# bqqbarbhg/rtk

Measured on AMD Instinct MI355X. Metric: Mrays/sec (primary, closest-hit) on 1M-tri scene, higher is better.
Workload: dtype f32; 1 GPU; config2: 1M-tri soup (seed 1, spread 0.02), 4096x4096 coherent pinhole primary rays; bvh=gpu-lbvh, bvh_nodes=462584, launch=persistent, ray_order=as given, parallelism=ray-batch shards x1, BVH replicated

## Files before the change

include/rtk_amd.h:

```cpp
#ifndef RTK_AMD_H
#define RTK_AMD_H

#include "rtk.h"

#ifdef __cplusplus
extern "C" {
#endif

enum {
	RTK_AMD_OK = 0,
	RTK_AMD_ERR_NO_DEVICE = -1,
	RTK_AMD_ERR_BAD_ARG = -2,
	RTK_AMD_ERR_OOM = -3,
	RTK_AMD_ERR_HIP = -4,
	RTK_AMD_ERR_BAD_SCENE = -5,
	RTK_AMD_ERR_UNSUPPORTED = -6,
};

const char *rtk_amd_last_error(void);
int rtk_amd_device_count(void);
int rtk_amd_set_device(int device);

typedef struct rtk_dev_scene rtk_dev_scene;

// ... 122 lines not shown
int rtk_dev_trace_status(const rtk_dev_scene *ds, void *stream);

int rtk_dev_detect_image(const rtk_dev_scene *ds, const rtk_ray *d_rays, size_t n, uint32_t *width, uint32_t *height, void *stream);

int rtk_dev_trace_rays_counted(const rtk_dev_scene *ds, const rtk_ray *d_rays, size_t n,
	rtk_hit_record *d_hits, const rtk_trace_opts *opts, rtk_trace_counters *out);

int rtk_dev_trace_rays_any_counted(const rtk_dev_scene *ds, const rtk_ray *d_rays, size_t n,
	uint8_t *d_occluded, const rtk_trace_opts *opts, rtk_trace_counters *out);

typedef struct rtk_packet_counters {
	uint64_t tiles;
	uint64_t pairs;
	uint64_t node_steps;
	uint64_t triangles_fetched;
	uint64_t triangle_group_tests;
	uint64_t tiles_handed_back;
	uint64_t handed_back_node_steps;
	uint64_t handed_back_triangle_steps;
} rtk_packet_counters;
int rtk_dev_trace_rays_packet_counted(const rtk_dev_scene *ds, const rtk_ray *d_rays, size_t n,
	rtk_hit_record *d_hits, const rtk_trace_opts *opts, rtk_packet_counters *out);

typedef struct rtk_mgpu rtk_mgpu;
void rtk_amd_shard_range(size_t n, int rank, int num_shards, size_t *first, size_t *count);
rtk_mgpu *rtk_mgpu_create(const int *devices, int num_devices);
void rtk_mgpu_destroy(rtk_mgpu *m);
int rtk_mgpu_num_devices(const rtk_mgpu *m);
const rtk_dev_scene *rtk_mgpu_scene(const rtk_mgpu *m, int index);
int rtk_mgpu_build(rtk_mgpu *m, const rtk_scene_desc *desc);
int rtk_mgpu_upload(rtk_mgpu *m, const rtk_scene *scene);
int rtk_mgpu_refit(rtk_mgpu *m, const rtk_scene_desc *desc);
int rtk_mgpu_refit_meshes(rtk_mgpu *m, const rtk_scene_desc *desc, const uint32_t *mesh_ids, size_t num_ids);
int rtk_mgpu_trace_rays(rtk_mgpu *m, const rtk_ray *rays, size_t n, rtk_hit_record *records, const rtk_trace_opts *opts);
int rtk_mgpu_trace_rays_device(rtk_mgpu *m, const rtk_ray *const *d_rays, const size_t *counts, rtk_hit_record *const *d_records,
	rtk_hit_record *d_gathered, int root_index, const rtk_trace_opts *opts);
int rtk_mgpu_trace_rays_device_striped(rtk_mgpu *m, const rtk_ray *const *d_rays, const size_t *counts, rtk_hit_record *const *d_records,
	rtk_hit_record *const *d_striped, const rtk_trace_opts *opts);
void rtk_mgpu_striped_segment(const size_t *counts, int num_shards, int shard, int stripe, size_t *first, size_t *count);

size_t rtk_trace_rays(const rtk_scene *scene, const rtk_ray *rays, size_t n, rtk_hit *hits, uint8_t *hit_mask);
size_t rtk_trace_rays_filter(const rtk_scene *scene, const rtk_ray *rays, size_t n, rtk_hit *hits, uint8_t *hit_mask,
	rtk_filter_fn *filter, void *filter_user);
void rtk_amd_forget_scene(const rtk_scene *scene);

#ifdef __cplusplus
// ... 4 lines not shown
```

rtk_amd/api.py:

```python
import ctypes as C
import os

import numpy as np

from .types import (HIT_DTYPE, HIT_RECORD_DTYPE, RAY_DTYPE, MeshSet, SceneDesc, SceneHeader)

HERE = os.path.dirname(os.path.abspath(__file__))
LIB_PATH = os.environ.get("RTK_AMD_LIB") or os.path.join(HERE, "librtk_amd.so")

RTK_TRACE_STATIC = 1
RTK_TRACE_NO_PACKET = 2
RTK_TRACE_SORT_RAYS = 4
RTK_TRACE_EXACT_NODES = 8
RTK_TRACE_NO_ASM = 16


class RtkError(RuntimeError):
    pass


class SceneInfo(C.Structure):
    _fields_ = [("num_triangles", C.c_uint64), ("num_meshes", C.c_uint64), ("num_nodes", C.c_uint64),
                ("node_bytes", C.c_uint64), ("triangle_bytes", C.c_uint64), ("total_device_bytes", C.c_uint64),
                ("max_depth", C.c_uint32), ("stack_entries", C.c_uint32), ("build_ms", C.c_double)]
# ... 49 lines not shown
    _fields_ = [("tiles", C.c_uint64), ("pairs", C.c_uint64), ("node_steps", C.c_uint64), ("triangles_fetched", C.c_uint64),
                ("triangle_group_tests", C.c_uint64), ("tiles_handed_back", C.c_uint64),
                ("handed_back_node_steps", C.c_uint64), ("handed_back_triangle_steps", C.c_uint64)]

    def as_dict(self):
        return {k: int(getattr(self, k)) for k, _ in self._fields_}


RTK_H_SYMBOLS = ["rtk_start_build", "rtk_run_task", "rtk_get_build_size", "rtk_finish_build_to",
                 "rtk_finish_build", "rtk_build_scene", "rtk_free_scene", "rtk_trace_ray", "rtk_trace_ray_filter"]
RTK_AMD_H_SYMBOLS = ["rtk_amd_last_error", "rtk_amd_device_count", "rtk_amd_set_device",
                     "rtk_dev_scene_upload", "rtk_dev_scene_build", "rtk_dev_scene_free", "rtk_dev_scene_get_info",
                     "rtk_dev_scene_mesh_base", "rtk_dev_scene_primitive_order", "rtk_dev_scene_export_size", "rtk_dev_scene_export",
                     "rtk_dev_trace_rays", "rtk_dev_trace_rays_any", "rtk_dev_expand_hits",
                     "rtk_dev_trace_rays_counted", "rtk_dev_trace_rays_any_counted", "rtk_dev_trace_rays_packet_counted", "rtk_dev_detect_image", "rtk_trace_rays", "rtk_amd_forget_scene",
                     "rtk_dev_scene_validate", "rtk_amd_release_workspace", "rtk_dev_scene_upload_buffer",
                     "rtk_dev_trace_rays_filtered", "rtk_dev_trace_rays_any_filtered", "rtk_dev_trace_status",
                     "rtk_trace_rays_filter", "rtk_amd_shard_range", "rtk_mgpu_create", "rtk_mgpu_destroy", "rtk_mgpu_num_devices",
                     "rtk_mgpu_scene", "rtk_mgpu_build", "rtk_mgpu_upload", "rtk_mgpu_trace_rays", "rtk_mgpu_trace_rays_device",
                     "rtk_amd_set_builder", "rtk_amd_get_builder", "rtk_amd_set_per_ray",
                     "rtk_mgpu_trace_rays_device_striped", "rtk_mgpu_striped_segment",
                     "rtk_dev_scene_refit", "rtk_dev_scene_last_refit_ms", "rtk_mgpu_refit",
                     "rtk_dev_scene_refit_meshes", "rtk_dev_scene_last_refit_nodes", "rtk_mgpu_refit_meshes",
                     "rtk_dev_scene_quality"]

_lib = None


def lib():
    global _lib
    if _lib is not None:
        return _lib
    if not os.path.exists(LIB_PATH):
        raise RtkError("%s not found: build it with `make -C rtk_amd/csrc` (or __graft_entry__.build()); "
                       "there is no CPU fallback" % LIB_PATH)
    import torch
    L = C.CDLL(LIB_PATH)
    L.rtk_amd_last_error.restype = C.c_char_p
    L.rtk_amd_device_count.restype = C.c_int
    L.rtk_amd_set_device.argtypes = [C.c_int]
    L.rtk_dev_scene_upload.restype = C.c_void_p
    L.rtk_dev_scene_upload.argtypes = [C.c_void_p]
    L.rtk_dev_scene_build.restype = C.c_void_p
    L.rtk_dev_scene_build.argtypes = [C.POINTER(SceneDesc)]
    L.rtk_dev_scene_free.argtypes = [C.c_void_p]
    L.rtk_dev_scene_get_info.argtypes = [C.c_void_p, C.POINTER(SceneInfo)]
    L.rtk_dev_scene_mesh_base.argtypes = [C.c_void_p, C.c_void_p, C.c_size_t]
    L.rtk_dev_scene_primitive_order.restype = C.c_longlong
    L.rtk_dev_scene_primitive_order.argtypes = [C.c_void_p, C.c_void_p, C.c_size_t]
    L.rtk_dev_scene_export_size.restype = C.c_size_t
    L.rtk_dev_scene_export_size.argtypes = [C.c_void_p]
    L.rtk_dev_scene_export.restype = C.c_void_p
    L.rtk_dev_scene_export.argtypes = [C.c_void_p, C.c_void_p, C.c_size_t]
    L.rtk_dev_trace_rays.argtypes = [C.c_void_p, C.c_void_p, C.c_size_t, C.c_void_p, C.POINTER(TraceOpts), C.c_void_p]
    L.rtk_dev_trace_rays_any.argtypes = [C.c_void_p, C.c_void_p, C.c_size_t, C.c_void_p, C.POINTER(TraceOpts), C.c_void_p]
    L.rtk_dev_expand_hits.argtypes = [C.c_void_p, C.c_void_p, C.c_size_t, C.c_void_p, C.c_void_p, C.c_void_p]
    L.rtk_dev_trace_rays_packet_counted.argtypes = [C.c_void_p, C.c_void_p, C.c_size_t, C.c_void_p, C.POINTER(TraceOpts), C.POINTER(PacketCounters)]
    L.rtk_dev_trace_rays_counted.argtypes = [C.c_void_p, C.c_void_p, C.c_size_t, C.c_void_p, C.POINTER(TraceOpts),
                                             C.POINTER(TraceCounters)]
    L.rtk_dev_trace_rays_any_counted.argtypes = [C.c_void_p, C.c_void_p, C.c_size_t, C.c_void_p, C.POINTER(TraceOpts),
                                                 C.POINTER(TraceCounters)]
    L.rtk_trace_rays.restype = C.c_size_t
    L.rtk_trace_rays.argtypes = [C.c_void_p, C.c_void_p, C.c_size_t, C.c_void_p, C.c_void_p]
    L.rtk_amd_forget_scene.argtypes = [C.c_void_p]
    L.rtk_dev_scene_validate.argtypes = [C.c_void_p, C.POINTER(SceneCheck)]
    L.rtk_dev_scene_upload_buffer.restype = C.c_void_p
    L.rtk_dev_scene_upload_buffer.argtypes = [C.c_void_p, C.c_size_t]
    L.rtk_dev_trace_rays_filtered.argtypes = [C.c_void_p, C.c_void_p, C.c_size_t, C.c_void_p, C.POINTER(DevFilter),
                                              C.POINTER(TraceOpts), C.c_void_p]
    L.rtk_dev_trace_rays_any_filtered.argtypes = [C.c_void_p, C.c_void_p, C.c_size_t, C.c_void_p, C.POINTER(DevFilter),
                                                  C.POINTER(TraceOpts), C.c_void_p]
    L.rtk_dev_trace_status.argtypes = [C.c_void_p, C.c_void_p]
    L.rtk_trace_rays_filter.restype = C.c_size_t
    L.rtk_trace_rays_filter.argtypes = [C.c_void_p, C.c_void_p, C.c_size_t, C.c_void_p, C.c_void_p, C.c_void_p, C.c_void_p]
    L.rtk_amd_shard_range.restype = None
    L.rtk_amd_shard_range.argtypes = [C.c_size_t, C.c_int, C.c_int, C.POINTER(C.c_size_t), C.POINTER(C.c_size_t)]
    L.rtk_mgpu_create.restype = C.c_void_p
    L.rtk_mgpu_create.argtypes = [C.POINTER(C.c_int), C.c_int]
    L.rtk_mgpu_destroy.restype = None
    L.rtk_mgpu_destroy.argtypes = [C.c_void_p]
# ... 309 lines not shown
        torch = _torch()
        if hasattr(rays, "data_ptr"):
            d_rays, n = rays, rays.numel() * rays.element_size() // 32
        else:
            rays = np.ascontiguousarray(rays)
            n = rays.shape[0]
            d_rays = to_device(rays)
        d_rec = torch.empty(n * 16, dtype=torch.uint8, device="cuda")
        ctr = TraceCounters()
        torch.cuda.synchronize()
        _check(lib().rtk_dev_trace_rays_counted(self.handle, C.c_void_p(d_rays.data_ptr()), n, C.c_void_p(d_rec.data_ptr()),
                                                C.byref(opts) if opts is not None else None, C.byref(ctr)),
               "rtk_dev_trace_rays_counted")
        return d_rec.cpu().numpy().view(HIT_RECORD_DTYPE), ctr.as_dict()


    def detect_image(self, rays):
        rays = np.ascontiguousarray(rays)
        d_rays = to_device(rays)
        w, h = C.c_uint32(0), C.c_uint32(0)
        _check(lib().rtk_dev_detect_image(self.handle, C.c_void_p(d_rays.data_ptr()), C.c_size_t(rays.shape[0]), C.byref(w), C.byref(h), _stream_ptr()), "rtk_dev_detect_image")
        return int(w.value), int(h.value)

    def trace_packet_counted(self, rays, opts):
        torch = _torch()
        if hasattr(rays, "data_ptr"):
            d_rays, n = rays, rays.numel() * rays.element_size() // 32
        else:
            rays = np.ascontiguousarray(rays)
            n = rays.shape[0]
            d_rays = to_device(rays)
        d_rec = torch.empty(n * 16, dtype=torch.uint8, device="cuda")
        ctr = PacketCounters()
        torch.cuda.synchronize()
        _check(lib().rtk_dev_trace_rays_packet_counted(self.handle, C.c_void_p(d_rays.data_ptr()), n, C.c_void_p(d_rec.data_ptr()),
                                                       C.byref(opts) if opts is not None else None, C.byref(ctr)),
               "rtk_dev_trace_rays_packet_counted")
        return d_rec.cpu().numpy().view(HIT_RECORD_DTYPE), ctr.as_dict()



def build_scene(meshes):
    _torch()
    ms = meshes if isinstance(meshes, MeshSet) else MeshSet(meshes)
    p = lib().rtk_build_scene(C.byref(ms.desc))
    if not p:
# ... 51 lines not shown
```

rtk_amd/csrc/rtk_capi.hip:

```cpp
#include "rtk_dev.h"
#include "rtk_trace_plan.h"

#include <algorithm>
#include "rtk_layout_check.h"

#include <stdarg.h>
#include <stdio.h>
#include <stdlib.h>
#include <string.h>

#include <chrono>
#include <atomic>
#include <mutex>
#include <unordered_map>


static thread_local char g_error[512] = "";

void rtk_set_error(const char *fmt, ...)
{
	va_list ap;
	va_start(ap, fmt);
	vsnprintf(g_error, sizeof(g_error), fmt, ap);
	va_end(ap);
// ... 105 lines not shown
{
	if (!out) { rtk_set_error("rtk_dev_trace_rays_counted: NULL counters"); return RTK_AMD_ERR_BAD_ARG; }
	return rtk_launch_trace(ds, d_rays, n, d_hits, nullptr, opts, nullptr, false, out);
}

extern "C" int rtk_dev_trace_rays_any_counted(const rtk_dev_scene *ds, const rtk_ray *d_rays, size_t n,
	uint8_t *d_occluded, const rtk_trace_opts *opts, rtk_trace_counters *out)
{
	if (!out) { rtk_set_error("rtk_dev_trace_rays_any_counted: NULL counters"); return RTK_AMD_ERR_BAD_ARG; }
	return rtk_launch_trace(ds, d_rays, n, nullptr, d_occluded, opts, nullptr, true, out);
}

extern "C" int rtk_dev_trace_rays_packet_counted(const rtk_dev_scene *ds, const rtk_ray *d_rays, size_t n,
	rtk_hit_record *d_hits, const rtk_trace_opts *opts, rtk_packet_counters *out)
{
	if (!out) { rtk_set_error("rtk_dev_trace_rays_packet_counted: NULL counters"); return RTK_AMD_ERR_BAD_ARG; }
	return rtk_launch_trace(ds, d_rays, n, d_hits, nullptr, opts, nullptr, false, nullptr, nullptr, nullptr, nullptr, 0, out);
}

extern "C" int rtk_dev_detect_image(const rtk_dev_scene *ds, const rtk_ray *d_rays, size_t n, uint32_t *width, uint32_t *height, void *stream)
{
	if (!ds || !width || !height || (!d_rays && n)) { rtk_set_error("rtk_dev_detect_image: NULL argument"); return RTK_AMD_ERR_BAD_ARG; }
	return rtk_detect_image(ds, d_rays, n, (hipStream_t)stream, width, height);
}

extern "C" int rtk_dev_trace_status(const rtk_dev_scene *ds, void *stream)
{
	return rtk_trace_status(ds, (hipStream_t)stream);
}

extern "C" int rtk_dev_expand_hits(const rtk_dev_scene *ds, const rtk_hit_record *d_records, size_t n,
	rtk_hit *d_hits, uint8_t *d_mask, void *stream)
{
	return rtk_launch_expand(ds, d_records, n, d_hits, d_mask, (hipStream_t)stream);
}


namespace {

const size_t STRIPE = 4096;

uint64_t hash_words(const void *data, size_t n, uint64_t h)
{
	const unsigned char *p = static_cast<const unsigned char *>(data);
	size_t i = 0;
	for (; i + 8 <= n; i += 8) { uint64_t w; memcpy(&w, p + i, 8); h = (h ^ w) * 0x9e3779b97f4a7c15ull; h ^= h >> 29; }
// ... 555 lines not shown
```

rtk_amd/csrc/rtk_dev.h:

```cpp
#pragma once

#include <hip/hip_runtime.h>
#include <stdint.h>
#include <mutex>
#include <vector>

#include "rtk.h"
#include "rtk_amd.h"

#define RTK_MAX_DEVICES 64
#define RTK_REF_NONE 0xffffffffu
#define RTK_REF_LEAF 0x80000000u
#define RTK_TRI_LAST 1u
#define RTK_QUEUES 8
#define RTK_QUEUE_WORD(q) (16 + 16 * (q))
#define RTK_COUNTER_WORDS (16 + 16 * RTK_QUEUES)
#define RTK_ERROR_WORD RTK_COUNTER_WORDS

struct DevNode {
	float bx[2][4];
	float by[2][4];
	float bz[2][4];
	uint32_t child[4];
	uint32_t order[4];
// ... 155 lines not shown
	WorkspaceLoan() = default;
	WorkspaceLoan(const WorkspaceLoan &) = delete;
	WorkspaceLoan &operator=(const WorkspaceLoan &) = delete;
	~WorkspaceLoan() { release(); }
	bool take(int device, size_t bytes);
	void release();
};
bool rtk_is_device_ptr(const void *p);
static inline size_t rtk_padded(size_t bytes) { return ((bytes ? bytes : 1) + 255u) & ~(size_t)255u; }
void rtk_export_forget(const rtk_dev_scene *ds);
void rtk_sah_costs(float *cost_node, float *cost_tri);

size_t rtk_sort_scratch_words(uint32_t n);
bool rtk_sort_pairs_async(unsigned long long *keys_a, unsigned long long *keys_b, uint32_t *vals_a, uint32_t *vals_b,
	uint32_t n, uint32_t key_bits, uint32_t *scratch, hipStream_t stream);
bool rtk_sort_words_async(unsigned long long *keys_a, unsigned long long *keys_b, uint32_t n, uint32_t first_bit, uint32_t last_bit,
	uint32_t *scratch, hipStream_t stream);

int rtk_launch_trace(const rtk_dev_scene *ds, const rtk_ray *d_rays, size_t n, rtk_hit_record *d_hits,
	uint8_t *d_occluded, const rtk_trace_opts *opts, hipStream_t stream, bool any_hit, rtk_trace_counters *counted,
	const rtk_dev_filter *filter = nullptr, rtk_hit_record *d_cand = nullptr, uint32_t *d_cand_count = nullptr, uint32_t cand_k = 0,
	rtk_packet_counters *pk_counted = nullptr);
int rtk_detect_image(const rtk_dev_scene *ds, const rtk_ray *d_rays, size_t n, hipStream_t stream, uint32_t *w_out, uint32_t *h_out);
int rtk_trace_status(const rtk_dev_scene *ds, hipStream_t stream);
void rtk_scratch_free(LaunchScratch *s);
void rtk_scene_drop_stream(rtk_dev_scene *ds, hipStream_t stream);
int rtk_launch_trace_one(const rtk_dev_scene *ds, const rtk_ray *d_ray, rtk_hit *d_hit, uint8_t *d_mask, hipStream_t stream,
	unsigned long long *h_status, uint32_t ticket);
int rtk_launch_expand(const rtk_dev_scene *ds, const rtk_hit_record *d_records, size_t n, rtk_hit *d_hits,
	uint8_t *d_mask, hipStream_t stream, unsigned long long *h_status = nullptr, uint32_t ticket = 0);
```

rtk_amd/csrc/rtk_trace.hip:

```cpp
#include "rtk_dev.h"

#include <algorithm>
#include "rtk_trace_shared.h"

#include <math.h>
#include <stdio.h>
#include <stdlib.h>

#include <mutex>

#include "rtk_trace_lane.h"

#define RTK_PUSH(e_)                                                                                        \
	do {                                                                                                    \
		if (sp < LDS_STACK) { stk[sp][lane] = (e_); sp++; }                                                 \
		else if (sp - LDS_STACK < p.spill_cap) {                                                            \
			p.spill[(size_t)(sp - LDS_STACK) * p.spill_stride + glane] = (e_); sp++; if (COUNT) c_spills++; \
		} else p.counter[RTK_ERROR_WORD] = 1ull;                                                            \
	} while (0)

#define RTK_REF_RETRY 0xfffffffeu
#define RTK_POP()                                                                                           \
	do {                                                                                                    \
		if (sp == 0u) top = RTK_REF_NONE;                                                                   \
// ... 802 lines not shown
#include "rtk_lane_hot_image.h"

const TraceKnobs &rtk_trace_knobs()
{
	static const TraceKnobs knobs = [] {
		const auto env = [](const char *name, int value) { const char *v = getenv(name); return v ? atoi(v) : value; };
		TraceKnobs k;
		k.detect_image = env("RTK_AMD_DETECT_IMAGE", k.detect_image);
		k.tile_blocks = env("RTK_AMD_TILE_BLOCKS", k.tile_blocks);
		k.any_packets = env("RTK_AMD_ANY_PACKETS", k.any_packets);
		k.qnodes = env("RTK_AMD_QNODES", k.qnodes);
		k.packet_asm = env("RTK_AMD_PACKET_ASM", k.packet_asm);
		const int wanted = env("RTK_AMD_PACKET_BEAM", (int)k.packet_beam);
		k.packet_beam = wanted < 0 ? PacketKernel::Cpp : wanted > (int)PacketKernel::Beam2 ? PacketKernel::Beam2 : (PacketKernel)wanted;
		k.log_path = getenv("RTK_AMD_LOG_PATH") != nullptr;
		k.lane_asm = env("RTK_AMD_LANE_ASM", k.lane_asm);
		k.lane_lds = (size_t)env("RTK_AMD_LANE_LDS", (int)k.lane_lds);
		k.sort_cell_bits = (uint32_t)env("RTK_AMD_SORT_CELL_BITS", (int)k.sort_cell_bits);
		k.sort_octant = (uint32_t)env("RTK_AMD_SORT_OCTANT", (int)k.sort_octant);
		k.sort_key = env("RTK_AMD_SORT_KEY", k.sort_key);
		k.packet_entries = env("RTK_AMD_PACKET_ENTRIES", k.packet_entries);
		k.entry_target = (unsigned)env("RTK_AMD_ENTRY_TARGET", (int)k.entry_target);
		k.entry_levels = (unsigned)env("RTK_AMD_ENTRY_LEVELS", (int)k.entry_levels);
		k.hot_blocks_per_cu = env("RTK_AMD_HOT_BLOCKS_PER_CU", k.hot_blocks_per_cu);
		k.lane_stats = env("RTK_AMD_LANE_STATS", k.lane_stats);
		k.lane_blocks = env("RTK_AMD_LANE_BLOCKS", k.lane_blocks);
		return k;
	}();
	return knobs;
}

AsmModule &rtk_lane_module()
{
	static const AsmKernel table[2] = { { "rtk_lane_hot_closest", rtk_trace_knobs().lane_blocks }, { "rtk_lane_hot_any", 0 } };
	static AsmModule m(rtk_lane_hot_image, table, 2, "rtk_dev_trace: the assembly per-lane kernels are not loaded");
	return m;
}

const AsmModule::Loaded *AsmModule::on(int device)
{
	if (device < 0 || device >= RTK_MAX_DEVICES) return nullptr;
	std::lock_guard<std::mutex> lock(mutex);
	Loaded &h = slot[device];
	if (!h.tried) {
		int cur = -1;
		if (hipGetDevice(&cur) != hipSuccess || cur != device) return nullptr;
// ... 271 lines not shown
	const int occ = blocks_per_cu_of(ds->device, variant_of(rq, o, look_w, look_h, facts, kernels, knobs));
	const TracePlan plan = plan_trace(rq, o, look_w, look_h, facts, kernels, knobs, occ);
	if (plan.error != RTK_AMD_OK) { rtk_set_error("%s", plan.message); return plan.error; }
	if (knobs.log_path) fprintf(stderr, "rtk_dev_trace: n %zu image %u x %u packet %d hot %d beam %d opts %p flags %x\n", n, plan.image_w, plan.image_h, (int)plan.packet, (int)plan.hot, (int)plan.kernel, (const void *)opts, o.flags);
	p.dynamic = plan.dynamic;
	p.refill_min = plan.refill_min;
	p.node_exit = plan.node_exit;
	p.image_w = plan.image_w;
	p.image_h = plan.image_h;
	p.tile_blocks = plan.tile_blocks;

	std::lock_guard<std::mutex> lock(ds->scratch_mutex);
	LaunchScratch *sc = scratch_for(ds, stream);
	if (!sc) return RTK_AMD_ERR_OOM;
	int rc = grow_scratch(sc, plan, n, stream);
	if (rc != RTK_AMD_OK) return rc;
	p.spill = sc->d_spill;
	p.spill_stride = (uint32_t)(plan.spill_cap ? sc->spill_lanes : 0);
	p.spill_cap = (uint32_t)plan.spill_cap;
	p.counter = sc->d_counter;
	if (plan.sort_rays && (rc = enqueue_sort(ds, sc, d_rays, n, knobs, stream, &p.perm)) != RTK_AMD_OK) return rc;
	if ((plan.dynamic || plan.packet || counted) && !plan.entries) RTK_HIP_CHECK(hipMemsetAsync(sc->d_counter, 0, RTK_COUNTER_WORDS * sizeof(unsigned long long), stream), RTK_AMD_ERR_HIP);
	if (plan.entries) {
		rtk_packet_entries_launch(p, (PkBlockEntries *)sc->d_entries, ds->bound_abs > 1.0f ? ds->bound_abs : 1.0f, knobs.entry_target, knobs.entry_levels, stream);
		p.entries = (const PkBlockEntries *)sc->d_entries;
	}
	if (plan.hot) rc = enqueue_packet_hot(ds, sc, p, plan, any_hit, pk_counted != nullptr, stream);
	else if (plan.packet) rtk_packet_launch(p, (unsigned)plan.grid, stream, counted != nullptr);
	else if (plan.lane_hot) rc = enqueue_lane_hot(ds, sc, p, plan, any_hit, o.refill_given, knobs, stream);
	else hipLaunchKernelGGL(trace_variant(plan.variant), dim3((unsigned)plan.grid), dim3(BLOCK_THREADS), 0, stream, p);
	if (rc != RTK_AMD_OK) return rc;
	RTK_HIP_CHECK(hipGetLastError(), RTK_AMD_ERR_HIP);
	if (pk_counted && (rc = read_packet_counters(sc, n, stream, pk_counted)) != RTK_AMD_OK) return rc;
	if (counted) return read_counters(sc, stream, counted);
	return RTK_AMD_OK;
}

int rtk_trace_status(const rtk_dev_scene *ds_c, hipStream_t stream)
{
	rtk_dev_scene *ds = const_cast<rtk_dev_scene *>(ds_c);
	if (!ds) { rtk_set_error("rtk_dev_trace_status: NULL scene"); return RTK_AMD_ERR_BAD_ARG; }
	unsigned long long *word = nullptr;
	{
		std::lock_guard<std::mutex> lock(ds->scratch_mutex);
		for (LaunchScratch *s : ds->scratch) if (s->stream == stream) { word = s->d_counter + RTK_ERROR_WORD; break; }
	}
	if (!word) {
		RTK_HIP_CHECK(hipStreamSynchronize(stream), RTK_AMD_ERR_HIP);
		return RTK_AMD_OK;
	}
	unsigned long long e = 0;
	RTK_HIP_CHECK(hipMemcpyAsync(&e, word, sizeof(e), hipMemcpyDeviceToHost, stream), RTK_AMD_ERR_HIP);
	RTK_HIP_CHECK(hipStreamSynchronize(stream), RTK_AMD_ERR_HIP);
	if (e) {
		(void)hipMemsetAsync(word, 0, sizeof(e), stream);
		rtk_set_error("rtk_dev_trace: traversal stack overflow (corrupted scene)");
		return RTK_AMD_ERR_BAD_SCENE;
// ... 50 lines not shown
```

rtk_amd/csrc/rtk_trace_packet.hip:

```cpp
#include "rtk_dev.h"
#include "rtk_trace_shared.h"

#include <math.h>

#define PK_LDS_STACK 16
#define PK_WAVE_STACK 64
#ifndef PK_MIN_WAVES
#define PK_MIN_WAVES 7
#endif

typedef int i32x16 __attribute__((ext_vector_type(16)));
typedef int i32x8 __attribute__((ext_vector_type(8)));
typedef int i32x4 __attribute__((ext_vector_type(4)));
typedef float f32x4 __attribute__((ext_vector_type(4)));

__device__ __forceinline__ float asf(int v) { return __int_as_float(v); }

struct PkNode { i32x4 nx, fx, ny, fy, nz, fz, ch; int ord; };
__device__ __forceinline__ void s_load_node(const char *addr, uint32_t onx, uint32_t ofx, uint32_t ony, uint32_t ofy,
	uint32_t onz, uint32_t ofz, uint32_t oord, PkNode &n)
{
	asm volatile(
		"s_load_dwordx4 %0, %8, %9\n\t"
		"s_load_dwordx4 %1, %8, %10\n\t"
// ... 468 lines not shown
		if (alive) {
			if (p.occluded) p.occluded[ray_index] = L.prim != RTK_PRIM_NONE ? 1 : 0;
			else {
				f32x4 rec;
				rec.x = L.t; rec.y = L.u; rec.z = L.v; rec.w = __uint_as_float(L.prim);
				__builtin_nontemporal_store(rec, reinterpret_cast<f32x4 *>(p.hits + ray_index));
			}
			if (COUNT) {
				atomicAdd(p.counter + 1, 1ull);
				atomicAdd(p.counter + 2, (unsigned long long)c_nodes);
				atomicAdd(p.counter + 3, (unsigned long long)c_leaves);
				atomicAdd(p.counter + 4, (unsigned long long)c_tris);
				atomicAdd(p.counter + 5, L.prim != RTK_PRIM_NONE ? 1ull : 0ull);
				atomicAdd(p.counter + 6, (unsigned long long)c_spills);
			}
		}
	}
}


namespace {
struct PkBeam { float olo[3], ohi[3], rlo[3], rhi[3], m[3], tmin; uint32_t neg; };

__device__ __forceinline__ bool pk_beam_child(const DevNode &nd, int k, const PkBeam &b, float &tlo)
{
	const float lo[3] = { nd.bx[0][k], nd.by[0][k], nd.bz[0][k] }, hi[3] = { nd.bx[1][k], nd.by[1][k], nd.bz[1][k] };
	float n = b.tmin, f = INFINITY;
#pragma unroll
	for (int a = 0; a < 3; a++) {
		const bool neg = (b.neg >> a) & 1u;
		const float pn = neg ? hi[a] : lo[a], pf = neg ? lo[a] : hi[a];
		const float n0 = (pn - b.olo[a]) * b.rlo[a], n1 = (pn - b.olo[a]) * b.rhi[a], n2 = (pn - b.ohi[a]) * b.rlo[a], n3 = (pn - b.ohi[a]) * b.rhi[a];
		const float f0 = (pf - b.olo[a]) * b.rlo[a], f1 = (pf - b.olo[a]) * b.rhi[a], f2 = (pf - b.ohi[a]) * b.rlo[a], f3 = (pf - b.ohi[a]) * b.rhi[a];
		n = fmaxf(n, fminf(fminf(n0, n1), fminf(n2, n3)) - b.m[a]);
		f = fminf(f, fmaxf(fmaxf(f0, f1), fmaxf(f2, f3)) + b.m[a]);
	}
	tlo = n;
	return n <= f;
}

__device__ __forceinline__ float wave_min(float v) { for (int o = 32; o > 0; o >>= 1) v = fminf(v, __shfl_xor(v, o)); return v; }
__device__ __forceinline__ float wave_max(float v) { for (int o = 32; o > 0; o >>= 1) v = fmaxf(v, __shfl_xor(v, o)); return v; }

#define PK_FRONTIER 128
__global__ void __launch_bounds__(64) rtk_packet_entries_kernel(const DevNode *nodes, const rtk_ray *rays, uint32_t image_w, uint32_t blocks_per_row,
	float bound_abs, uint32_t target, uint32_t max_levels, PkBlockEntries *out, unsigned long long *counter)
{
	__shared__ uint32_t s_ref[2][PK_FRONTIER];
	if (blockIdx.x == 0) for (uint32_t w = threadIdx.x; w < (uint32_t)RTK_COUNTER_WORDS; w += 64u) counter[w] = 0ull;
	__shared__ float s_t[2][PK_FRONTIER];
	__shared__ uint32_t s_out_ref[PK_MAX_ENTRIES];
	__shared__ float s_out_t[PK_MAX_ENTRIES];
	const uint32_t lane = threadIdx.x, blk = blockIdx.x;
	const uint32_t bx = blk % blocks_per_row, by = blk / blocks_per_row;
	PkBeam b;
	bool ok = true;
	uint32_t s_and = 7u, s_or = 0u;
	float tmin = INFINITY;
	for (int a = 0; a < 3; a++) { b.olo[a] = INFINITY; b.ohi[a] = -INFINITY; b.rlo[a] = INFINITY; b.rhi[a] = -INFINITY; }
	if (lane < 9u) {
		const uint32_t x = (lane % 3u) == 0u ? 0u : ((lane % 3u) == 1u ? 31u : 63u);
		const uint32_t y = (lane / 3u) == 0u ? 0u : ((lane / 3u) == 1u ? 31u : 63u);
		const rtk_ray r = rays[(size_t)(by * 64u + y) * image_w + bx * 64u + x];
		const float o[3] = { r.origin.x, r.origin.y, r.origin.z }, d[3] = { r.direction.x, r.direction.y, r.direction.z };
		uint32_t sg = 0;
		for (int a = 0; a < 3; a++) {
			const float rd = 1.0f / d[a];
			ok = ok && fabsf(o[a]) < 0x1p19f && fabsf(rd) > 0x1p-100f && fabsf(rd) < 0x1p100f;
// ... 62 lines not shown
		}
		over = over || n_out > PK_MAX_ENTRIES || n_next > PK_FRONTIER;
		if (over) break;
		__syncthreads();
		cur ^= 1u;
		n_cur = n_next;
	}
	if (!over) {
		for (uint32_t i = lane; i < n_cur; i += 64u) if (n_out + i < PK_MAX_ENTRIES) { s_out_ref[n_out + i] = s_ref[cur][i]; s_out_t[n_out + i] = s_t[cur][i]; }
		n_out += n_cur;
		over = n_out > PK_MAX_ENTRIES;
	}
	__syncthreads();
	if (over) { if (lane == 0) e->count = 0u; return; }
	if (lane < n_out) {
		const float t = s_out_t[lane];
		uint32_t rank = 0;
		for (uint32_t j = 0; j < n_out; j++) { const float tj = s_out_t[j]; rank += (tj < t || (tj == t && j < lane)) ? 1u : 0u; }
		e->e[rank].ref = s_out_ref[lane];
		e->e[rank].tlo = t;
	}
	if (lane == 0) e->count = n_out;
}
}

void rtk_packet_entries_launch(const TraceParams &p, PkBlockEntries *out, float bound_abs, unsigned target, unsigned max_levels, hipStream_t stream)
{
	const uint32_t bpr = p.image_w >> 6, rows = p.image_h >> 6;
	hipLaunchKernelGGL(rtk_packet_entries_kernel, dim3(bpr * rows), dim3(64), 0, stream, p.sc.nodes, p.rays, p.image_w, bpr, bound_abs, target, max_levels, out, p.counter);
}

#include "rtk_packet_hot_image.h"

AsmModule &rtk_packet_module()
{
	static const AsmKernel table[NUM_PACKET_KERNELS] = {
		{ "rtk_packet_hot", 7 },
		{ "rtk_packet_beam", 8 },
		{ "rtk_packet_beam2", 7 },
		{ "rtk_packet_count2", 0 },
		{ "rtk_packet_any2", 0 },
	};
	static AsmModule m(rtk_packet_hot_image, table, NUM_PACKET_KERNELS, "rtk_dev_trace: the assembly packet kernel is not loaded");
	return m;
}

int rtk_packet_occupancy(bool counted)
{
	int nb = 0;
	hipError_t e = counted ? hipOccupancyMaxActiveBlocksPerMultiprocessor(&nb, rtk_trace_packet_kernel<true>, TRACE_BLOCK_THREADS, 0)
	                       : hipOccupancyMaxActiveBlocksPerMultiprocessor(&nb, rtk_trace_packet_kernel<false>, TRACE_BLOCK_THREADS, 0);
	return (e == hipSuccess && nb >= 1) ? nb : 1;
// ... 8 lines not shown
```

rtk_amd/csrc/rtk_trace_plan.h:

```cpp
#pragma once

#include "rtk_amd.h"

#include <stddef.h>
#include <stdint.h>

#ifndef LDS_STACK
#define LDS_STACK 15
#endif
#define TRACE_WAVES_PER_BLOCK 4
#define TRACE_BLOCK_THREADS (64 * TRACE_WAVES_PER_BLOCK)

enum { VARIANT_COLLECT = 16, VARIANT_PACKET = 18, VARIANT_PACKET_COUNTED = 19, NUM_VARIANTS = 20 };

enum class PacketKernel { Cpp = -1, Hot, Beam, Beam2, Count2, Any2 };
enum { NUM_PACKET_KERNELS = 5 };

struct TraceKnobs {
	int detect_image = 1;
	int tile_blocks = 1;
	int any_packets = 1;
	int qnodes = 1;
	int packet_asm = 1;
	PacketKernel packet_beam = PacketKernel::Beam2;
	bool log_path = false;
	int lane_asm = 1;
	size_t lane_lds = LDS_STACK;
	uint32_t sort_cell_bits = 7u;
	uint32_t sort_octant = 0u;
	int sort_key = 1;
	int packet_entries = 1;
	unsigned entry_target = 26u;
	unsigned entry_levels = 8u;
	int hot_blocks_per_cu = 0;
	int lane_stats = 0;
	int lane_blocks = 5;
};

const TraceKnobs &rtk_trace_knobs();

struct TraceOpts {
	uint32_t flags = 0;
	uint32_t image_w = 0, image_h = 0;
	uint32_t refill_min = 0;
	uint32_t blocks_per_cu = 0;
	uint32_t node_exit = 0;
	bool refill_given = false;
};

inline TraceOpts decode_opts(const rtk_trace_opts *opts)
{
	TraceOpts o;
	if (!opts || opts->struct_size < 16) return o;
	o.flags = opts->flags;
	o.image_w = opts->image_width;
	o.image_h = opts->image_height;
// ... 159 lines not shown
```

rtk_amd/csrc/rtk_trace_shared.h:

```cpp
#pragma once

#include "rtk_dev.h"
#include "rtk_trace_plan.h"

#include <stddef.h>
#include <mutex>

#define WAVES_PER_BLOCK TRACE_WAVES_PER_BLOCK
#define BLOCK_THREADS TRACE_BLOCK_THREADS

struct TraceParams {
	DevSceneView sc;
	const rtk_ray *rays;
	rtk_hit_record *hits;
	uint8_t *occluded;
	unsigned long long *counter;
	uint2 *spill;
	unsigned long long n;
	uint32_t spill_stride;
	uint32_t spill_cap;
	uint32_t image_w, image_h;
	uint32_t refill_min;
	uint32_t dynamic;
	uint32_t node_exit;
// ... 74 lines not shown
	const unsigned long long tile = i >> 6;
	const uint32_t in = (uint32_t)i & 63u;
	const uint32_t tiles_per_row = w >> 3;
	unsigned long long ty;
	uint32_t tx;
	if (blocks) {
		const unsigned long long blk = tile >> 6;
		const uint32_t b = (uint32_t)tile & 63u, blocks_per_row = w >> 6;
		const unsigned long long by = blk / blocks_per_row;
		tx = (uint32_t)(blk - by * blocks_per_row) * 8u + (b & 7u);
		ty = by * 8u + (b >> 3);
	} else {
		ty = tile / tiles_per_row;
		tx = (uint32_t)(tile - ty * tiles_per_row);
	}
	const unsigned long long x = (unsigned long long)tx * 8u + (in & 7u);
	const unsigned long long y = ty * 8u + (in >> 3);
	return y * w + x;
}


int rtk_packet_occupancy(bool counted);
void rtk_packet_launch(const TraceParams &p, unsigned blocks, hipStream_t stream, bool counted);
void rtk_packet_entries_launch(const TraceParams &p, PkBlockEntries *out, float bound_abs, unsigned target, unsigned max_levels, hipStream_t stream);

struct AsmKernel {
	const char *name;
	int cap;
};
struct AsmModule {
	enum { MAX_KERNELS = NUM_PACKET_KERNELS };
	struct Loaded { hipModule_t mod = nullptr; hipFunction_t fn[MAX_KERNELS] = {}; int blocks_per_cu[MAX_KERNELS] = {}; bool tried = false; };
	const void *image;
	const AsmKernel *table;
	int count;
	const char *not_loaded;
	std::mutex mutex;
	Loaded slot[RTK_MAX_DEVICES];
	AsmModule(const void *image_, const AsmKernel *table_, int count_, const char *not_loaded_) : image(image_), table(table_), count(count_), not_loaded(not_loaded_) {}
	const Loaded *on(int device);
	int launch(int device, int kernel, void *params, size_t size, unsigned blocks, hipStream_t stream);
};
AsmModule &rtk_lane_module();
AsmModule &rtk_packet_module();
```

Measured before the change: 25180 Mrays/s.

## Rewrite per-block beam entry-list kernel to process four child slots per wave

Adds a new beam entry-list builder kernel, made the default through a knob, that maps the wave's 64 lanes to 16 frontier nodes times 4 child slots. It walks up to 64 frontier nodes per chunk and uses ballots and popcounts to compact leaf entries and pushed children. The old kernel stays available through an env knob. A debug API to dump entry lists is added, and the final sort is done by rank computed from lane reads. This targets the setup cost of the entries pre-pass before the hot packet kernel, at the price of more register use and more complex code.

```diff
diff --git a/include/rtk_amd.h b/include/rtk_amd.h
--- a/include/rtk_amd.h
+++ b/include/rtk_amd.h
@@ -168,6 +168,9 @@
 int rtk_dev_trace_rays_packet_counted(const rtk_dev_scene *ds, const rtk_ray *d_rays, size_t n,
 	rtk_hit_record *d_hits, const rtk_trace_opts *opts, rtk_packet_counters *out);
 
+int rtk_dev_packet_entries_debug(const rtk_dev_scene *ds, const rtk_ray *d_rays, size_t n, const rtk_trace_opts *opts,
+	void *out_host, size_t out_bytes);
+
 typedef struct rtk_mgpu rtk_mgpu;
 void rtk_amd_shard_range(size_t n, int rank, int num_shards, size_t *first, size_t *count);
 rtk_mgpu *rtk_mgpu_create(const int *devices, int num_devices);
diff --git a/rtk_amd/api.py b/rtk_amd/api.py
--- a/rtk_amd/api.py
+++ b/rtk_amd/api.py
@@ -95,7 +95,7 @@
                      "rtk_mgpu_trace_rays_device_striped", "rtk_mgpu_striped_segment",
                      "rtk_dev_scene_refit", "rtk_dev_scene_last_refit_ms", "rtk_mgpu_refit",
                      "rtk_dev_scene_refit_meshes", "rtk_dev_scene_last_refit_nodes", "rtk_mgpu_refit_meshes",
-                     "rtk_dev_scene_quality"]
+                     "rtk_dev_scene_quality", "rtk_dev_packet_entries_debug"]
 
 _lib = None
 
@@ -129,6 +129,8 @@
     L.rtk_dev_trace_rays_any.argtypes = [C.c_void_p, C.c_void_p, C.c_size_t, C.c_void_p, C.POINTER(TraceOpts), C.c_void_p]
     L.rtk_dev_expand_hits.argtypes = [C.c_void_p, C.c_void_p, C.c_size_t, C.c_void_p, C.c_void_p, C.c_void_p]
     L.rtk_dev_trace_rays_packet_counted.argtypes = [C.c_void_p, C.c_void_p, C.c_size_t, C.c_void_p, C.POINTER(TraceOpts), C.POINTER(PacketCounters)]
+    L.rtk_dev_packet_entries_debug.restype = C.c_int
+    L.rtk_dev_packet_entries_debug.argtypes = [C.c_void_p, C.c_void_p, C.c_size_t, C.POINTER(TraceOpts), C.c_void_p, C.c_size_t]
     L.rtk_dev_trace_rays_counted.argtypes = [C.c_void_p, C.c_void_p, C.c_size_t, C.c_void_p, C.POINTER(TraceOpts),
                                              C.POINTER(TraceCounters)]
     L.rtk_dev_trace_rays_any_counted.argtypes = [C.c_void_p, C.c_void_p, C.c_size_t, C.c_void_p, C.POINTER(TraceOpts),
@@ -484,6 +486,17 @@
         _check(lib().rtk_dev_detect_image(self.handle, C.c_void_p(d_rays.data_ptr()), C.c_size_t(rays.shape[0]), C.byref(w), C.byref(h), _stream_ptr()), "rtk_dev_detect_image")
         return int(w.value), int(h.value)
 
+    def packet_entries_debug(self, rays, opts):
+        torch = _torch()
+        rays = np.ascontiguousarray(rays)
+        d_rays = to_device(rays)
+        blocks = (int(opts.image_width) // 64) * (int(opts.image_height) // 64)
+        out = np.zeros((max(blocks, 1), 512), np.uint8)
+        torch.cuda.synchronize()
+        _check(lib().rtk_dev_packet_entries_debug(self.handle, C.c_void_p(d_rays.data_ptr()), C.c_size_t(rays.shape[0]), C.byref(opts),
+                                                  C.c_void_p(out.ctypes.data), C.c_size_t(out.nbytes)), "rtk_dev_packet_entries_debug")
+        return out[:blocks]
+
     def trace_packet_counted(self, rays, opts):
         torch = _torch()
         if hasattr(rays, "data_ptr"):
diff --git a/rtk_amd/csrc/rtk_capi.hip b/rtk_amd/csrc/rtk_capi.hip
--- a/rtk_amd/csrc/rtk_capi.hip
+++ b/rtk_amd/csrc/rtk_capi.hip
@@ -151,6 +151,11 @@
 {
 	if (!ds || !width || !height || (!d_rays && n)) { rtk_set_error("rtk_dev_detect_image: NULL argument"); return RTK_AMD_ERR_BAD_ARG; }
 	return rtk_detect_image(ds, d_rays, n, (hipStream_t)stream, width, height);
+}
+
+extern "C" int rtk_dev_packet_entries_debug(const rtk_dev_scene *ds, const rtk_ray *d_rays, size_t n, const rtk_trace_opts *opts, void *out_host, size_t out_bytes)
+{
+	return rtk_packet_entries_debug(ds, d_rays, n, opts, out_host, out_bytes);
 }
 
 extern "C" int rtk_dev_trace_status(const rtk_dev_scene *ds, void *stream)
diff --git a/rtk_amd/csrc/rtk_dev.h b/rtk_amd/csrc/rtk_dev.h
--- a/rtk_amd/csrc/rtk_dev.h
+++ b/rtk_amd/csrc/rtk_dev.h
@@ -201,6 +201,7 @@
 	const rtk_dev_filter *filter = nullptr, rtk_hit_record *d_cand = nullptr, uint32_t *d_cand_count = nullptr, uint32_t cand_k = 0,
 	rtk_packet_counters *pk_counted = nullptr);
 int rtk_detect_image(const rtk_dev_scene *ds, const rtk_ray *d_rays, size_t n, hipStream_t stream, uint32_t *w_out, uint32_t *h_out);
+int rtk_packet_entries_debug(const rtk_dev_scene *ds, const rtk_ray *d_rays, size_t n, const rtk_trace_opts *opts, void *out_host, size_t out_bytes);
 int rtk_trace_status(const rtk_dev_scene *ds, hipStream_t stream);
 void rtk_scratch_free(LaunchScratch *s);
 void rtk_scene_drop_stream(rtk_dev_scene *ds, hipStream_t stream);
diff --git a/rtk_amd/csrc/rtk_trace.hip b/rtk_amd/csrc/rtk_trace.hip
--- a/rtk_amd/csrc/rtk_trace.hip
+++ b/rtk_amd/csrc/rtk_trace.hip
@@ -848,6 +848,7 @@
 		k.packet_entries = env("RTK_AMD_PACKET_ENTRIES", k.packet_entries);
 		k.entry_target = (unsigned)env("RTK_AMD_ENTRY_TARGET", (int)k.entry_target);
 		k.entry_levels = (unsigned)env("RTK_AMD_ENTRY_LEVELS", (int)k.entry_levels);
+		k.entries_kernel = env("RTK_AMD_ENTRIES_KERNEL", k.entries_kernel);
 		k.hot_blocks_per_cu = env("RTK_AMD_HOT_BLOCKS_PER_CU", k.hot_blocks_per_cu);
 		k.lane_stats = env("RTK_AMD_LANE_STATS", k.lane_stats);
 		k.lane_blocks = env("RTK_AMD_LANE_BLOCKS", k.lane_blocks);
@@ -1165,7 +1166,7 @@
 	if (plan.sort_rays && (rc = enqueue_sort(ds, sc, d_rays, n, knobs, stream, &p.perm)) != RTK_AMD_OK) return rc;
 	if ((plan.dynamic || plan.packet || counted) && !plan.entries) RTK_HIP_CHECK(hipMemsetAsync(sc->d_counter, 0, RTK_COUNTER_WORDS * sizeof(unsigned long long), stream), RTK_AMD_ERR_HIP);
 	if (plan.entries) {
-		rtk_packet_entries_launch(p, (PkBlockEntries *)sc->d_entries, ds->bound_abs > 1.0f ? ds->bound_abs : 1.0f, knobs.entry_target, knobs.entry_levels, stream);
+		rtk_packet_entries_launch(p, (PkBlockEntries *)sc->d_entries, ds->bound_abs > 1.0f ? ds->bound_abs : 1.0f, knobs.entry_target, knobs.entry_levels, knobs.entries_kernel, stream);
 		p.entries = (const PkBlockEntries *)sc->d_entries;
 	}
 	if (plan.hot) rc = enqueue_packet_hot(ds, sc, p, plan, any_hit, pk_counted != nullptr, stream);
@@ -1176,6 +1177,43 @@
 	RTK_HIP_CHECK(hipGetLastError(), RTK_AMD_ERR_HIP);
 	if (pk_counted && (rc = read_packet_counters(sc, n, stream, pk_counted)) != RTK_AMD_OK) return rc;
 	if (counted) return read_counters(sc, stream, counted);
+	return RTK_AMD_OK;
+}
+
+int rtk_packet_entries_debug(const rtk_dev_scene *ds_c, const rtk_ray *d_rays, size_t n, const rtk_trace_opts *opts, void *out_host, size_t out_bytes)
+{
+	rtk_dev_scene *ds = const_cast<rtk_dev_scene *>(ds_c);
+	if (!ds || !d_rays || !out_host) { rtk_set_error("rtk_dev_packet_entries_debug: NULL argument"); return RTK_AMD_ERR_BAD_ARG; }
+	const TraceOpts o = decode_opts(opts);
+	TraceRequest rq;
+	rq.n = n;
+	if (!hinted_image(rq, o) || !whole_blocks(o.image_w, o.image_h) || n > 0x40000000ull) {
+		rtk_set_error("rtk_dev_packet_entries_debug: the options must name an image of whole 64x64-pixel blocks that is this batch");
+		return RTK_AMD_ERR_BAD_ARG;
+	}
+	if (!(ds->bound_abs < 0x1p19f) || ds->view.num_nodes == 0u) { rtk_set_error("rtk_dev_packet_entries_debug: no entry lists are made for this scene"); return RTK_AMD_ERR_UNSUPPORTED; }
+	const size_t nblk = (size_t)(o.image_w >> 6) * (o.image_h >> 6);
+	if (out_bytes < nblk * sizeof(PkBlockEntries)) { rtk_set_error("rtk_dev_packet_entries_debug: %zu blocks need %zu bytes", nblk, nblk * sizeof(PkBlockEntries)); return RTK_AMD_ERR_BAD_ARG; }
+	if (!on_scene_device(ds, "rtk_dev_packet_entries_debug")) return RTK_AMD_ERR_BAD_ARG;
+	const TraceKnobs &knobs = rtk_trace_knobs();
+	hipStream_t stream = nullptr;
+	std::lock_guard<std::mutex> lock(ds->scratch_mutex);
+	LaunchScratch *sc = scratch_for(ds, stream);
+	if (!sc) return RTK_AMD_ERR_OOM;
+	const int rc = grow(&sc->d_entries, &sc->entries_capacity, nblk, nblk * sizeof(PkBlockEntries), stream);
+	if (rc != RTK_AMD_OK) return rc;
+	TraceParams p = {};
+	p.sc = ds->view;
+	p.rays = d_rays;
+	p.n = n;
+	p.image_w = o.image_w;
+	p.image_h = o.image_h;
+	p.counter = sc->d_counter;
+	RTK_HIP_CHECK(hipMemsetAsync(sc->d_entries, 0, nblk * sizeof(PkBlockEntries), stream), RTK_AMD_ERR_HIP);
+	rtk_packet_entries_launch(p, (PkBlockEntries *)sc->d_entries, ds->bound_abs > 1.0f ? ds->bound_abs : 1.0f, knobs.entry_target, knobs.entry_levels, knobs.entries_kernel, stream);
+	RTK_HIP_CHECK(hipGetLastError(), RTK_AMD_ERR_HIP);
+	RTK_HIP_CHECK(hipMemcpyAsync(out_host, sc->d_entries, nblk * sizeof(PkBlockEntries), hipMemcpyDeviceToHost, stream), RTK_AMD_ERR_HIP);
+	RTK_HIP_CHECK(hipStreamSynchronize(stream), RTK_AMD_ERR_HIP);
 	return RTK_AMD_OK;
 }
 
diff --git a/rtk_amd/csrc/rtk_trace_packet.hip b/rtk_amd/csrc/rtk_trace_packet.hip
--- a/rtk_amd/csrc/rtk_trace_packet.hip
+++ b/rtk_amd/csrc/rtk_trace_packet.hip
@@ -514,9 +514,8 @@
 namespace {
 struct PkBeam { float olo[3], ohi[3], rlo[3], rhi[3], m[3], tmin; uint32_t neg; };
 
-__device__ __forceinline__ bool pk_beam_child(const DevNode &nd, int k, const PkBeam &b, float &tlo)
-{
-	const float lo[3] = { nd.bx[0][k], nd.by[0][k], nd.bz[0][k] }, hi[3] = { nd.bx[1][k], nd.by[1][k], nd.bz[1][k] };
+__device__ __forceinline__ bool pk_beam_box(const float (&lo)[3], const float (&hi)[3], const PkBeam &b, float &tlo)
+{
 	float n = b.tmin, f = INFINITY;
 #pragma unroll
 	for (int a = 0; a < 3; a++) {
@@ -531,11 +530,17 @@
 	return n <= f;
 }
 
+__device__ __forceinline__ bool pk_beam_child(const DevNode &nd, int k, const PkBeam &b, float &tlo)
+{
+	const float lo[3] = { nd.bx[0][k], nd.by[0][k], nd.bz[0][k] }, hi[3] = { nd.bx[1][k], nd.by[1][k], nd.bz[1][k] };
+	return pk_beam_box(lo, hi, b, tlo);
+}
+
 __device__ __forceinline__ float wave_min(float v) { for (int o = 32; o > 0; o >>= 1) v = fminf(v, __shfl_xor(v, o)); return v; }
 __device__ __forceinline__ float wave_max(float v) { for (int o = 32; o > 0; o >>= 1) v = fmaxf(v, __shfl_xor(v, o)); return v; }
 
 #define PK_FRONTIER 128
-__global__ void __launch_bounds__(64) rtk_packet_entries_kernel(const DevNode *nodes, const rtk_ray *rays, uint32_t image_w, uint32_t blocks_per_row,
+__global__ void __launch_bounds__(64) rtk_packet_entries_kernel_v1(const DevNode *nodes, const rtk_ray *rays, uint32_t image_w, uint32_t blocks_per_row,
 	float bound_abs, uint32_t target, uint32_t max_levels, PkBlockEntries *out, unsigned long long *counter)
 {
 	__shared__ uint32_t s_ref[2][PK_FRONTIER];
@@ -644,12 +649,169 @@
 	}
 	if (lane == 0) e->count = n_out;
 }
-}
-
-void rtk_packet_entries_launch(const TraceParams &p, PkBlockEntries *out, float bound_abs, unsigned target, unsigned max_levels, hipStream_t stream)
+
+
+__device__ __forceinline__ float lane_value(float v, int l) { return __uint_as_float((uint32_t)__builtin_amdgcn_readlane((int)__float_as_uint(v), l)); }
+__device__ __forceinline__ float nine_min(float v) { float r = lane_value(v, 0); for (int l = 1; l < 9; l++) r = fminf(r, lane_value(v, l)); return r; }
+__device__ __forceinline__ float nine_max(float v) { float r = lane_value(v, 0); for (int l = 1; l < 9; l++) r = fmaxf(r, lane_value(v, l)); return r; }
+
+template <int NSUB>
+__device__ __forceinline__ void pk_entries_chunk(const DevNode *nodes, const PkBeam &b, const uint32_t *f_ref, const float *f_t, uint32_t cnt, uint32_t lane,
+	uint32_t *nx_ref, float *nx_t, uint32_t *o_ref, float *o_t, uint32_t &n_out, uint32_t &n_next)
+{
+	const uint32_t k = lane >> 4, i = lane & 15u;
+	uint32_t ref[NSUB], child[NSUB];
+	float t_self[NSUB], lo[NSUB][3], hi[NSUB][3];
+	bool have[NSUB];
+#pragma unroll
+	for (int s = 0; s < NSUB; s++) {
+		const uint32_t j = (uint32_t)s * 16u + i;
+		have[s] = j < cnt;
+		ref[s] = have[s] ? f_ref[j] : 0u;
+		t_self[s] = have[s] ? f_t[j] : 0.0f;
+	}
+#pragma unroll
+	for (int s = 0; s < NSUB; s++) {
+		const DevNode &nd = nodes[ref[s]];
+		lo[s][0] = nd.bx[0][k]; hi[s][0] = nd.bx[1][k];
+		lo[s][1] = nd.by[0][k]; hi[s][1] = nd.by[1][k];
+		lo[s][2] = nd.bz[0][k]; hi[s][2] = nd.bz[1][k];
+		child[s] = nd.child[k];
+	}
+	unsigned long long L[NSUB], P[NSUB];
+	bool list[NSUB], push[NSUB];
+	float tlo[NSUB];
+#pragma unroll
+	for (int s = 0; s < NSUB; s++) {
+		tlo[s] = 0.0f;
+		const bool pass = have[s] && child[s] != RTK_REF_NONE && pk_beam_box(lo[s], hi[s], b, tlo[s]);
+		const unsigned long long m_leaf = __builtin_amdgcn_ballot_w64(pass && (child[s] & RTK_REF_LEAF) != 0u);
+		L[s] = (m_leaf | (m_leaf >> 16) | (m_leaf >> 32) | (m_leaf >> 48)) & 0xffffull;
+		list[s] = ((L[s] >> i) & 1ull) != 0ull;
+		push[s] = pass && !list[s];
+		P[s] = __builtin_amdgcn_ballot_w64(push[s]);
+	}
+	uint32_t listed = 0u;
+#pragma unroll
+	for (int s = 0; s < NSUB; s++) {
+		if (list[s] && k == 0u) {
+			const uint32_t at = n_out + listed + (uint32_t)__popcll(L[s] & ((1ull << i) - 1ull));
+			if (at < PK_MAX_ENTRIES) { o_ref[at] = ref[s]; o_t[at] = t_self[s]; }
+		}
+		listed += (uint32_t)__popcll(L[s]);
+	}
+	n_out += listed;
+	const unsigned long long row = 0xffffull << (16u * k), rows_below = (1ull << (16u * k)) - 1ull, lanes_below = (1ull << lane) - 1ull;
+	uint32_t before = 0u, pushed = 0u;
+#pragma unroll
+	for (int s = 0; s < NSUB; s++) before += (uint32_t)__popcll(P[s] & rows_below);
+#pragma unroll
+	for (int s = 0; s < NSUB; s++) {
+		if (push[s]) {
+			const uint32_t at = n_next + before + (uint32_t)__popcll(P[s] & row & lanes_below);
+			if (at < PK_FRONTIER) { nx_ref[at] = child[s]; nx_t[at] = tlo[s]; }
+		}
+		before += (uint32_t)__popcll(P[s] & row);
+		pushed += (uint32_t)__popcll(P[s]);
+	}
+	n_next += pushed;
+}
+
+__global__ void __launch_bounds__(64) rtk_packet_entries_kernel(const DevNode *nodes, const rtk_ray *rays, uint32_t image_w, uint32_t blocks_per_row,
+	float bound_abs, uint32_t target, uint32_t max_levels, PkBlockEntries *out, unsigned long long *counter)
+{
+	__shared__ uint32_t s_ref[2][PK_FRONTIER];
+	__shared__ float s_t[2][PK_FRONTIER];
+	__shared__ uint32_t s_out_ref[64];
+	__shared__ float s_out_t[64];
+	if (blockIdx.x == 0) for (uint32_t w = threadIdx.x; w < (uint32_t)RTK_COUNTER_WORDS; w += 64u) counter[w] = 0ull;
+	const uint32_t lane = threadIdx.x, blk = blockIdx.x;
+	const uint32_t bx = blk % blocks_per_row, by = blk / blocks_per_row;
+	float o[3] = { 0.0f, 0.0f, 0.0f }, rd[3] = { 0.0f, 0.0f, 0.0f }, tmin = 0.0f;
+	uint32_t sg = 0u;
+	bool ok = true;
+	if (lane < 9u) {
+		const uint32_t x = (lane % 3u) == 0u ? 0u : ((lane % 3u) == 1u ? 31u : 63u);
+		const uint32_t y = (lane / 3u) == 0u ? 0u : ((lane / 3u) == 1u ? 31u : 63u);
+		const rtk_ray r = rays[(size_t)(by * 64u + y) * image_w + bx * 64u + x];
+		const float ro[3] = { r.origin.x, r.origin.y, r.origin.z }, d[3] = { r.direction.x, r.direction.y, r.direction.z };
+		for (int a = 0; a < 3; a++) {
+			o[a] = ro[a];
+			rd[a] = 1.0f / d[a];
+			ok = ok && fabsf(o[a]) < 0x1p19f && fabsf(rd[a]) > 0x1p-100f && fabsf(rd[a]) < 0x1p100f;
+			sg |= (__float_as_uint(d[a]) >> 31) << a;
+		}
+		ok = ok && r.min_t == r.min_t && r.max_t == r.max_t;
+		tmin = r.min_t;
+	}
+	PkBeam b;
+	b.neg = 0u;
+	bool one_sign = true;
+	for (int a = 0; a < 3; a++) {
+		const unsigned long long m = __builtin_amdgcn_ballot_w64(lane < 9u && ((sg >> a) & 1u) != 0u);
+		b.neg |= (m != 0ull ? 1u : 0u) << a;
+		one_sign = one_sign && (m == 0ull || m == 0x1ffull);
+	}
+	ok = __builtin_amdgcn_ballot_w64(!ok) == 0ull && one_sign && bound_abs < 0x1p19f;
+	for (int a = 0; a < 3; a++) {
+		b.olo[a] = nine_min(o[a]); b.ohi[a] = nine_max(o[a]); b.rlo[a] = nine_min(rd[a]); b.rhi[a] = nine_max(rd[a]);
+		b.rlo[a] -= 0x1p-22f * fabsf(b.rlo[a]); b.rhi[a] += 0x1p-22f * fabsf(b.rhi[a]);
+		b.m[a] = 0x1p-21f * (fmaxf(fabsf(b.rlo[a]), fabsf(b.rhi[a])) * (fmaxf(fabsf(b.olo[a]), fabsf(b.ohi[a])) + bound_abs));
+	}
+	b.tmin = nine_min(tmin);
+	PkBlockEntries *e = out + blk;
+	if (lane == 0) {
+		for (int a = 0; a < 3; a++) { e->olo[a] = b.olo[a]; e->ohi[a] = b.ohi[a]; e->rlo[a] = b.rlo[a]; e->rhi[a] = b.rhi[a]; }
+		e->pad[0] = __float_as_uint(b.tmin); e->pad[1] = 0u; e->pad[2] = 0u;
+		if (!ok) e->count = 0u;
+	}
+	if (!ok) return;
+	uint32_t n_cur = 1u, n_out = 0u, cur = 0u;
+	bool over = false;
+	if (lane == 0) { s_ref[0][0] = 0u; s_t[0][0] = b.tmin; }
+	__syncthreads();
+	for (int level = 0; level < (int)max_levels && n_cur != 0u; level++) {
+		if (level > 0 && n_out + n_cur >= target) break;
+		uint32_t n_next = 0u;
+		for (uint32_t base = 0; base < n_cur; base += 64u) {
+			const uint32_t cnt = n_cur - base < 64u ? n_cur - base : 64u;
+			const uint32_t *f_ref = s_ref[cur] + base;
+			const float *f_t = s_t[cur] + base;
+			if (cnt <= 16u) pk_entries_chunk<1>(nodes, b, f_ref, f_t, cnt, lane, s_ref[cur ^ 1u], s_t[cur ^ 1u], s_out_ref, s_out_t, n_out, n_next);
+			else if (cnt <= 32u) pk_entries_chunk<2>(nodes, b, f_ref, f_t, cnt, lane, s_ref[cur ^ 1u], s_t[cur ^ 1u], s_out_ref, s_out_t, n_out, n_next);
+			else pk_entries_chunk<4>(nodes, b, f_ref, f_t, cnt, lane, s_ref[cur ^ 1u], s_t[cur ^ 1u], s_out_ref, s_out_t, n_out, n_next);
+		}
+		over = over || n_out > PK_MAX_ENTRIES || n_next > PK_FRONTIER;
+		if (over) break;
+		__syncthreads();
+		cur ^= 1u;
+		n_cur = n_next;
+	}
+	if (!over) {
+		for (uint32_t i = lane; i < n_cur; i += 64u) if (n_out + i < PK_MAX_ENTRIES) { s_out_ref[n_out + i] = s_ref[cur][i]; s_out_t[n_out + i] = s_t[cur][i]; }
+		n_out += n_cur;
+		over = n_out > PK_MAX_ENTRIES;
+	}
+	__syncthreads();
+	if (over) { if (lane == 0) e->count = 0u; return; }
+	const bool mine = lane < n_out;
+	const float t = mine ? s_out_t[lane] : 0.0f;
+	const uint32_t ref = mine ? s_out_ref[lane] : 0u;
+	uint32_t rank = 0;
+	for (uint32_t j = 0; j < n_out; j++) { const float tj = lane_value(t, (int)j); rank += (tj < t || (tj == t && j < lane)) ? 1u : 0u; }
+	if (mine) {
+		e->e[rank].ref = ref;
+		e->e[rank].tlo = t;
+	}
+	if (lane == 0) e->count = n_out;
+}
+}
+
+void rtk_packet_entries_launch(const TraceParams &p, PkBlockEntries *out, float bound_abs, unsigned target, unsigned max_levels, int kernel, hipStream_t stream)
 {
 	const uint32_t bpr = p.image_w >> 6, rows = p.image_h >> 6;
-	hipLaunchKernelGGL(rtk_packet_entries_kernel, dim3(bpr * rows), dim3(64), 0, stream, p.sc.nodes, p.rays, p.image_w, bpr, bound_abs, target, max_levels, out, p.counter);
+	if (kernel == 0) hipLaunchKernelGGL(rtk_packet_entries_kernel_v1, dim3(bpr * rows), dim3(64), 0, stream, p.sc.nodes, p.rays, p.image_w, bpr, bound_abs, target, max_levels, out, p.counter);
+	else hipLaunchKernelGGL(rtk_packet_entries_kernel, dim3(bpr * rows), dim3(64), 0, stream, p.sc.nodes, p.rays, p.image_w, bpr, bound_abs, target, max_levels, out, p.counter);
 }
 
 #include "rtk_packet_hot_image.h"
diff --git a/rtk_amd/csrc/rtk_trace_plan.h b/rtk_amd/csrc/rtk_trace_plan.h
--- a/rtk_amd/csrc/rtk_trace_plan.h
+++ b/rtk_amd/csrc/rtk_trace_plan.h
@@ -32,6 +32,7 @@
 	int packet_entries = 1;
 	unsigned entry_target = 26u;
 	unsigned entry_levels = 8u;
+	int entries_kernel = 1;
 	int hot_blocks_per_cu = 0;
 	int lane_stats = 0;
 	int lane_blocks = 5;
diff --git a/rtk_amd/csrc/rtk_trace_shared.h b/rtk_amd/csrc/rtk_trace_shared.h
--- a/rtk_amd/csrc/rtk_trace_shared.h
+++ b/rtk_amd/csrc/rtk_trace_shared.h
@@ -120,7 +120,7 @@
 
 int rtk_packet_occupancy(bool counted);
 void rtk_packet_launch(const TraceParams &p, unsigned blocks, hipStream_t stream, bool counted);
-void rtk_packet_entries_launch(const TraceParams &p, PkBlockEntries *out, float bound_abs, unsigned target, unsigned max_levels, hipStream_t stream);
+void rtk_packet_entries_launch(const TraceParams &p, PkBlockEntries *out, float bound_abs, unsigned target, unsigned max_levels, int kernel, hipStream_t stream);
 
 struct AsmKernel {
 	const char *name;
```

Measured after the change: 25270 Mrays/s, median of 2. About the same (+0.3%).
